# cocowy1/Cost-Volume-Aggregation-in-Stereo-Matching-Revisited

Hardware: AMD Instinct MI355X
Metric: cost-volumes/sec (fwd+bwd) at 544x960 D=192 (higher is better)
Workload: dtype f32

## Files before the change

### cost-volume-aggregation-in-stereo-matching-revisited_amd/csrc/conv3d_c1.hip

```cpp
#include "dca_common.h"
#include "../../include/dca_hip.h"

namespace {
constexpr int TD = 4, TH = 8, TW = 32, CK = 4;
constexpr int ID = TD + 2, IH = TH + 2, IWP = 40;

struct C1Args {
  const float* x;
  const float* w;
  const float* dy;
  float* out;
  int N, C, D, H, W;
  int nTD, nTH, nTW, ntiles;
  int vec;
};

__device__ __forceinline__ void stage_tile(const float* __restrict__ src, float* lds, int n, int C, int c0, int nch,
                                           int D, int H, int W, int d0, int h0, int w0, int vec, int tid) {
  const int rows = nch * ID * IH;
  if (vec) {
    for (int it = tid; it < rows * 8; it += 256) {
      const int row = it >> 3, q = it & 7;
      const int c = row / (ID * IH), rem = row % (ID * IH), id = rem / IH, ih = rem % IH;
      const int ci = c0 + c, d = d0 - 1 + id, h = h0 - 1 + ih, wq = w0 + 4 * q;
// ... 20 lines not shown
      if (ci < C && (unsigned)d < (unsigned)D && (unsigned)h < (unsigned)H && (unsigned)wi < (unsigned)W)
        v = src[((((long)n * C + ci) * D + d) * H + h) * W + wi];
      lds[row * IWP + 3 + j] = v;
    }
  }
}

__device__ __forceinline__ void tile_coords(const C1Args& a, int tile, int& n, int& d0, int& h0, int& w0) {
  const int tw = tile % a.nTW; tile /= a.nTW;
  const int th = tile % a.nTH; tile /= a.nTH;
  const int td = tile % a.nTD;
  n = tile / a.nTD;
  d0 = td * TD; h0 = th * TH; w0 = tw * TW;
}

__global__ __launch_bounds__(256) void c1_bwd_data_kernel(C1Args a) {
  __shared__ __attribute__((aligned(16))) float dy_lds[ID * IH * IWP];
  extern __shared__ __attribute__((aligned(16))) float w_lds[];
  const int tid = threadIdx.x, wq = tid & 7, row = tid >> 3, dl = row >> 3, hl = row & 7;
  int n, d0, h0, w0;
  tile_coords(a, xcd_remap(blockIdx.x, gridDim.x), n, d0, h0, w0);
  stage_tile(a.dy, dy_lds, n, 1, 0, 1, a.D, a.H, a.W, d0, h0, w0, a.vec, tid);
  for (int i = tid; i < a.C * 27; i += 256) {
    const int c = i / 27, t = i % 27;
    w_lds[(c * 9 + t / 3) * 4 + t % 3] = a.w[c * 27 + 26 - t];
  }
  __syncthreads();
  float g[9][6];
#pragma unroll
  for (int r9 = 0; r9 < 9; ++r9) {
    const float* p = dy_lds + ((dl + r9 / 3) * IH + hl + r9 % 3) * IWP + 4 * wq;
    const float4 v = *(const float4*)(p + 4);
    g[r9][0] = p[3]; g[r9][1] = v.x; g[r9][2] = v.y; g[r9][3] = v.z; g[r9][4] = v.w; g[r9][5] = p[8];
  }
  const int d = d0 + dl, h = h0 + hl, w = w0 + 4 * wq;
  const bool ok = d < a.D && h < a.H && w < a.W;
  for (int c = 0; c < a.C; ++c) {
    float acc[4] = {0.f, 0.f, 0.f, 0.f};
#pragma unroll
    for (int r9 = 0; r9 < 9; ++r9) {
      const float4 wv = *(const float4*)(w_lds + (c * 9 + r9) * 4);
#pragma unroll
      for (int j = 0; j < 4; ++j)
        acc[j] = fmaf(wv.z, g[r9][j + 2], fmaf(wv.y, g[r9][j + 1], fmaf(wv.x, g[r9][j], acc[j])));
    }
    if (ok) {
      float* o = a.out + ((((long)n * a.C + c) * a.D + d) * a.H + h) * a.W + w;
      if (a.vec) {
        *(float4*)o = make_float4(acc[0], acc[1], acc[2], acc[3]);
      } else {
#pragma unroll
        for (int j = 0; j < 4; ++j)
          if (w + j < a.W) o[j] = acc[j];
      }
    }
  }
}

__global__ __launch_bounds__(256) void c1_gather_kernel(const float* __restrict__ T, float* __restrict__ y, int D, int H,
                                                        int W) {
  const long DHW = (long)D * H * W;
  const long n = blockIdx.y;
  const float* p = T + n * 27 * DHW;
  const long end = min(DHW, ((long)blockIdx.x + 1) * 1024);
  for (long idx = (long)blockIdx.x * 1024 + threadIdx.x; idx < end; idx += 256) {
    const int w = idx % W;
    const int t = (int)(idx / W);
    const int h = t % H, d = t / H;
    float s = 0.f;
#pragma unroll
// ... 53 lines not shown
      for (int j = 0; j < 4; ++j) v[j] = dca_bload1(dr, base + 4 * j, okr & (int)((unsigned)(w0 + j) < (unsigned)W));
    }
    *(float4*)(out + 4 * (long)q) = make_float4(v[0], v[1], v[2], v[3]);
  }
}

int fill_args(C1Args& a, int N, int C, int D, int H, int W, const void* p0, const void* p1, const void* p2) {
  a.N = N; a.C = C; a.D = D; a.H = H; a.W = W;
  a.nTD = cdiv(D, TD); a.nTH = cdiv(H, TH); a.nTW = cdiv(W, TW);
  const long nt = (long)N * a.nTD * a.nTH * a.nTW;
  if (nt >= (1L << 31)) return 1;
  a.ntiles = (int)nt;
  a.vec = (W % 4 == 0) && ((((uintptr_t)p0 | (uintptr_t)p1 | (uintptr_t)p2) & 15) == 0);
  return 0;
}
}

extern "C" int dca_conv3d_c1_bwd_data(const float* dy, const float* w, float* dx, int N, int C, int D, int H, int W,
                                      hipStream_t stream) {
  DCA_REQUIRE(dy && w && dx && N > 0 && C > 0 && C <= 256 && D > 0 && H > 0 && W > 0);
  C1Args a;
  a.x = nullptr; a.w = w; a.dy = dy; a.out = dx;
  DCA_REQUIRE(fill_args(a, N, C, D, H, W, dy, dx, nullptr) == 0);
  hipLaunchKernelGGL(c1_bwd_data_kernel, dim3(a.ntiles), dim3(256), (size_t)C * 36 * 4, stream, a);
  return dca_launch_status();
}

extern "C" int dca_conv3d_c1_gather(const float* T, float* y, int N, int D, int H, int W, hipStream_t stream) {
  DCA_REQUIRE(T && y && N > 0 && D > 0 && H > 0 && W > 0);
  DCA_REQUIRE(9L * D * H * W * 4 < 0x7ffffff0L && N <= 65535);
// ... 15 lines not shown
```

### cost-volume-aggregation-in-stereo-matching-revisited_amd/csrc/dca_common.h

```cpp
#pragma once
#include <hip/hip_runtime.h>
#include <stdint.h>
#include "../../include/dca_hip.h"

typedef float f32x16 __attribute__((ext_vector_type(16)));
typedef float f32x4 __attribute__((ext_vector_type(4)));

#define DCA_WAVE 64

#define DCA_REQUIRE(cond)                      \
  do {                                         \
    if (!(cond)) return (int)hipErrorInvalidValue; \
  } while (0)

static inline int dca_launch_status() { return (int)hipGetLastError(); }

static inline int cdiv(long a, long b) { return (int)((a + b - 1) / b); }

static inline int dca_num_cus() {
  int dev = 0, v = 0;
  if (hipGetDevice(&dev) == hipSuccess && hipDeviceGetAttribute(&v, hipDeviceAttributeMultiprocessorCount, dev) == hipSuccess &&
      v > 0)
    return v;
  return 256;
}
static inline int dca_persistent_grid(long tiles, int share) {
  const int ncu = dca_num_cus(), g = ncu > share ? ncu / share : 1;
  return (int)(tiles < g ? tiles : g);
}
int dca_internal_wgrad_reduce(const float* part, float* dw, int nblk, int nCxT, int nCT, int K, int Cy, int Cx, long s_cy,
                              long s_cx, hipStream_t stream);

__device__ __forceinline__ int xcd_remap(int bid, int nwg) {
  const int q = nwg >> 3, r = nwg & 7, xcd = bid & 7, idx = bid >> 3;
  const int base = (xcd < r) ? xcd * (q + 1) : r * (q + 1) + (xcd - r) * q;
  return base + idx;
}

__device__ __forceinline__ float act_apply(float v, float slope) { return v > 0.f ? v : v * slope; }

__device__ __forceinline__ float wave_sum(float v) {
#pragma unroll
  for (int o = 32; o > 0; o >>= 1) v += __shfl_xor(v, o, 64);
  return v;
}
__device__ __forceinline__ double wave_sum_d(double v) {
#pragma unroll
  for (int o = 32; o > 0; o >>= 1) v += __shfl_xor(v, o, 64);
  return v;
}
__device__ __forceinline__ float wave_max(float v) {
#pragma unroll
  for (int o = 32; o > 0; o >>= 1) v = fmaxf(v, __shfl_xor(v, o, 64));
  return v;
// ... 65 lines not shown
```

### cost-volume-aggregation-in-stereo-matching-revisited_amd/csrc/dca_frag.h

```cpp
#pragma once
#include "dca_common.h"

typedef __bf16 bf16x8 __attribute__((ext_vector_type(8)));
typedef _Float16 f16x8 __attribute__((ext_vector_type(8)));
typedef _Float16 f16x4 __attribute__((ext_vector_type(4)));
typedef short s16x4 __attribute__((__vector_size__(4 * sizeof(short))));
typedef short s16x8 __attribute__((__vector_size__(8 * sizeof(short))));
typedef __attribute__((address_space(3))) s16x4 lds_s16x4;

template <typename MT> struct Lp;
template <> struct Lp<__bf16> {
  typedef bf16x8 vec8;
  static __device__ __forceinline__ f32x16 mfma(vec8 a, vec8 b, f32x16 c) {
    return __builtin_amdgcn_mfma_f32_32x32x16_bf16(a, b, c, 0, 0, 0);
  }
};
template <> struct Lp<_Float16> {
  typedef f16x8 vec8;
  static __device__ __forceinline__ f32x16 mfma(vec8 a, vec8 b, f32x16 c) {
    return __builtin_amdgcn_mfma_f32_32x32x16_f16(a, b, c, 0, 0, 0);
  }
};
template <typename MT> __device__ __forceinline__ unsigned short lp_bits(float v) {
  const MT m = (MT)v;
// ... 8 lines not shown
template <typename MT> __device__ __forceinline__ float lp_hi(unsigned w) {
  return (float)__builtin_bit_cast(MT, (unsigned short)(w >> 16));
}
template <typename MT> __device__ __forceinline__ unsigned lp_pack2(float a, float b) {
  typedef float f32x2 __attribute__((ext_vector_type(2)));
  typedef MT mtx2 __attribute__((ext_vector_type(2)));
  const f32x2 v = {a, b};
  return __builtin_bit_cast(unsigned, __builtin_convertvector(v, mtx2));
}

__device__ __forceinline__ void x2_split(float v, int e, _Float16& h, _Float16& l) {
  const float u = ldexpf(v, e);
  h = (_Float16)u;
  l = (_Float16)(u - (float)h);
}

__device__ __forceinline__ void x2_prep_exps(int* xe, int A, const unsigned* __restrict__ slots, int nslots,
                                             int* __restrict__ xexps, int xexps_given) {
  const int tid = threadIdx.x;
  if (slots && !xexps_given) {
    for (int c0 = 0; c0 < A; c0 += 32) {
      const int c = c0 + (tid >> 4), l = tid & 15;
      unsigned v = 0;
      if (c < A)
        for (int i = l; i < nslots; i += 16) { const unsigned u = slots[(long)c * DCA_AMAX_CSLOTS + i]; v = v > u ? v : u; }
#pragma unroll
      for (int o = 8; o > 0; o >>= 1) { const unsigned u = (unsigned)__shfl_xor((int)v, o, 64); v = v > u ? v : u; }
      if (c < A && l == 0) {
        const int e = x2_scale_exp(v);
        xe[c] = e;
// ... 96 lines not shown
```

### cost-volume-aggregation-in-stereo-matching-revisited_amd/csrc/pointwise.hip

```cpp
#include "dca_frag.h"
#include "../../include/dca_hip.h"

__global__ __launch_bounds__(256) void bn_stats_kernel(const float* __restrict__ x, double* __restrict__ part, int N,
                                                       int C, long S, int nchunk, long chunk_len, int vec) {
  const int c = blockIdx.x, ch = blockIdx.y, tid = threadIdx.x;
  const long s0 = ch * chunk_len, s1 = min(S, s0 + chunk_len);
  const float K = x[(long)c * S];
  if (ch == 0 && tid == 0) part[(long)C * nchunk * 2 + c] = (double)K;
  float s = 0.f, ss = 0.f;
  for (int n = 0; n < N; ++n) {
    const float* p = x + ((long)n * C + c) * S;
    if (vec) {
      for (long i = s0 + 4 * tid; i < s1; i += 1024) {
        float4 v = *(const float4*)(p + i);
        v.x -= K; v.y -= K; v.z -= K; v.w -= K;
        s += (v.x + v.y) + (v.z + v.w);
        ss += (v.x * v.x + v.y * v.y) + (v.z * v.z + v.w * v.w);
      }
    } else {
      for (long i = s0 + tid; i < s1; i += 256) {
        const float v = p[i] - K;
        s += v;
        ss += v * v;
      }
// ... 135 lines not shown
        const float yv = y[base + i];
        ym = fmaxf(ym, fabsf(yv - mean));
        float v = yv * sc + sh;
        if (res_pre) v += res_pre[base + i];
        v = act_apply(v, slope);
        if (res_post) v += res_post[base + i];
        z[base + i] = v;
        am = fmaxf(am, fabsf(v));
      }
    }
  }
  if (zmax) dca_cmax_put(am, zmax + (long)c * DCA_AMAX_CSLOTS + ch);
  if (ymax) dca_cmax_put(ym, ymax + (long)c * DCA_AMAX_CSLOTS + ch);
}

__device__ __forceinline__ void px2_split(float v, int e, unsigned short& h, unsigned short& l) {
  _Float16 hh, ll;
  x2_split(v, e, hh, ll);
  h = __builtin_bit_cast(unsigned short, hh);
  l = __builtin_bit_cast(unsigned short, ll);
}
typedef unsigned short u16x8 __attribute__((ext_vector_type(8)));

__global__ __launch_bounds__(256) void bn_apply_pack_kernel(const float* __restrict__ y, const float* __restrict__ stats,
                                                            const int* __restrict__ zexps, char* __restrict__ zp, int N,
                                                            int C, long S, long chunk_len, float slope,
                                                            unsigned* __restrict__ ymax, const float* __restrict__ res_pre,
                                                            const float* __restrict__ res_post, float* __restrict__ zf,
                                                            unsigned* __restrict__ zmax) {
  const int cg = blockIdx.y, ch = blockIdx.x, tid = threadIdx.x;
  const long s0 = ch * chunk_len, s1 = min(S, s0 + chunk_len);
  float mean[8], sc[8], sh[8], ym[8], zm[8];
  int ex[8];
#pragma unroll
  for (int j = 0; j < 8; ++j) {
    const int c = cg * 8 + j;
    mean[j] = stats ? stats[c] : 0.f;
    sc[j] = stats ? stats[2 * C + c] : 1.f;
// ... 278 lines not shown
    k1[j] = training ? dca_coherent_loadf(dgb + 2 * C + c) : 0.f;
    k2[j] = training ? dca_coherent_loadf(dgb + 3 * C + c) * stats[C + c] : 0.f;
    ex[j] = dca_coherent_loadi(dyexps + c);
  }
  const long tb = px2_term_bytes(C, S);
  for (int n = 0; n < N; ++n) {
    const long base = ((long)n * C + cg * 8) * S;
    char* ob = dyp + (long)n * 2 * tb + (long)cg * S * 16;
    for (long i = s0 + tid; i < s1; i += 256) {
      float yv[8], dv[8];
#pragma unroll
      for (int j = 0; j < 8; ++j) { yv[j] = y[base + j * S + i]; dv[j] = dz[base + j * S + i]; }
      u16x8 hv, lv;
#pragma unroll
      for (int j = 0; j < 8; ++j) {
        const float u = yv[j] * sc[j] + sh[j];
        const float g = dv[j] * (u > 0.f ? 1.f : slope);
        const float o = (g - k1[j] - (yv[j] - mean[j]) * k2[j]) * sc[j];
        unsigned short h, l;
        px2_split(o, ex[j], h, l);
        hv[j] = h; lv[j] = l;
      }
      *(u16x8*)(ob + i * 16) = hv;
      *(u16x8*)(ob + tb + i * 16) = lv;
    }
  }
}

__global__ __launch_bounds__(256) void avgpool3d_fwd_kernel(const float* __restrict__ x, float* __restrict__ y, int Di,
                                                            int Hi, int Wi, int Do, int Ho, int Wo) {
  const long row = blockIdx.x;
  const int od = (int)(row % Do);
  const long nc = row / Do;
// ... 488 lines not shown
}

extern "C" int dca_bn_backward_reduce(const float* dz, const float* y, const float* stats, double* part, float* dgb, int N,
                                      int C, long S, float slope, int training, hipStream_t stream) {
  DCA_REQUIRE(dz && y && stats && part && dgb && N > 0 && C > 0 && S > 0 && C <= 65535);
  int nchunk; long len;
  chunking(S, C, &nchunk, &len);
  const int vec = (S % 4 == 0) && ((((uintptr_t)dz | (uintptr_t)y) & 15) == 0);
  hipLaunchKernelGGL(bn_bwd_reduce_kernel, dim3(C, nchunk), dim3(256), 0, stream, dz, y, (const float*)nullptr, stats, part,
                     N, C, S, nchunk, len, slope, vec, (unsigned*)nullptr);
  hipLaunchKernelGGL(bn_bwd_finalize_kernel, dim3(C), dim3(64), 0, stream, part, nchunk, (double)N * (double)S, dgb, C,
                     stats, training, (const unsigned*)nullptr, (const unsigned*)nullptr, 0, (int*)nullptr);
  return dca_launch_status();
}

extern "C" int dca_bn_backward_pack(const float* dz, const float* y, const float* stats, double* part, float* dgb, void* dyp,
                                    int* dyexps, unsigned* gmax, const unsigned* ymax, int ymax_slots, int N, int C, long S,
                                    float slope, int training, hipStream_t stream) {
  DCA_REQUIRE(dz && y && stats && part && dgb && dyp && dyexps && gmax && N > 0 && C > 0 && C % 8 == 0 && S > 0 && C <= 65535);
  DCA_REQUIRE((ymax == nullptr || (ymax_slots > 0 && ymax_slots <= DCA_AMAX_CSLOTS)) && ((((uintptr_t)dyp) & 15) == 0));
  int nchunk; long len;
  chunking(S, C, &nchunk, &len);
  const uintptr_t al = (uintptr_t)dz | (uintptr_t)y;
  const int vec = (S % 4 == 0) && ((al & 15) == 0);
  hipLaunchKernelGGL(bn_bwd_reduce_kernel, dim3(C, nchunk), dim3(256), 0, stream, dz, y, (const float*)nullptr, stats, part,
                     N, C, S, nchunk, len, slope, vec, gmax);
  hipLaunchKernelGGL(bn_bwd_finalize_kernel, dim3(C), dim3(64), 0, stream, part, nchunk, (double)N * (double)S, dgb, C,
                     stats, training, (const unsigned*)gmax, ymax, ymax_slots, dyexps);
  int pchunk; long plen;
  chunking(S, C / 8, &pchunk, &plen);
// ... 66 lines not shown
```

### cost-volume-aggregation-in-stereo-matching-revisited_amd/models/augment/cva.py

```python
import torch
import torch.nn as nn

from .._bootstrap import ensure as _ensure
from ..submodule import ConvBn3d, ConvBnReLU3d, conv3d_plain, convbn_3d
from .semantic_level import SemanticLevelContext

ops = _ensure().ops


class _DeconvBn3d(nn.Sequential):

    def __init__(self, cin, cout):
        super().__init__(nn.ConvTranspose3d(cin, cout, 3, padding=1, output_padding=1, stride=2, bias=False),
                         nn.BatchNorm3d(cout))

    def forward(self, x, slope=1.0, res_pre=None, res_post=None, pack_out=False):
        return ops.convbn3d(x, self[0], self[1], slope, res_pre, res_post, pack_out=pack_out)


class Multi_Aggregation(nn.Module):

    def __init__(self, in_channels):
        super().__init__()
        self.conv1 = ConvBnReLU3d(in_channels, in_channels * 2, 3, 2, 1)
# ... 14 lines not shown
        super().__init__(nn.AvgPool3d((3, 3, 3), stride=2, padding=1), ConvBn3d(32, 32, 3, 1, 1),
                         nn.ReLU(inplace=True))

    def forward(self, x):
        return self[1](ops.avg_pool3d_k3s2p1(x), slope=0.0)


class _Classify(nn.Sequential):

    def __init__(self, c):
        super().__init__(ConvBn3d(c, c, 3, 1, 1), nn.ReLU(inplace=True),
                         nn.Conv3d(c, 1, kernel_size=3, padding=1, stride=1, bias=False))

    def forward(self, x, alias=False):
        if alias:
            h, xa = self[0](x, slope=0.0, alias=True)
            return conv3d_plain(h, self[2]), xa
        h = self[0](x, slope=0.0)
        if h.dtype != torch.float32:
            return ops.conv3d_c1_lp(h, self[2].weight)
        return conv3d_plain(h, self[2])


class cva(nn.Module):

    def __init__(self, max_disp, in_channel, downsample=True):
        super().__init__()
        self.max_disp = max_disp
        self.channel = in_channel
        if downsample:
            self.downsample = _Downsample()
        self.slc_net = SemanticLevelContext(feats_channels=self.channel, transform_channels=self.channel,
# ... 44 lines not shown
```

### cost-volume-aggregation-in-stereo-matching-revisited_amd/ops.py

```python
from __future__ import annotations

import ctypes
import math
import os
import threading
from typing import Optional

import torch

from . import _lib

_C = _lib.CONSTANTS
_vp = ctypes.c_void_p


def _L():
    return _lib.load()


def _ptr(t: Optional[torch.Tensor]):
    return _vp(t.data_ptr()) if t is not None else None


_raw_stream = getattr(torch._C, "_cuda_getCurrentRawStream", None)
# ... 256 lines not shown


def _round_up(a, m):
    return (a + m - 1) // m * m


_CONV_MODE = os.environ.get("DCA_CONV", "x2")
CONV_X3 = _CONV_MODE != "fp32"
CONV_X2 = _CONV_MODE == "x2"
WGRAD_S2_X2 = os.environ.get("DCA_WGRAD_S2", "x2") != "fp32"
DECONV_X3 = os.environ.get("DCA_DECONV", "x3") != "fp32"
C1_WGRAD_FUSED = os.environ.get("DCA_C1_WGRAD", "fused") != "expand"
CONV_S2_X2 = os.environ.get("DCA_CONV_S2", "x2") != "fp32"
BN_FUSE = os.environ.get("DCA_BN_FUSE", "1") != "0"
C1_BWD_FUSE = os.environ.get("DCA_C1_BWD", "fused") != "split"
_X3_MIN_WORKGROUPS = 1


AMAX_STATS = {"tagged": 0, "computed": 0, "packed": 0}
CSLOTS = _C["DCA_AMAX_CSLOTS"]
AMAX_EMIT = os.environ.get("DCA_AMAX_EMIT", "1") != "0"
PACK = os.environ.get("DCA_PACK", "1") != "0"


def _cslots(C, device):
    if not AMAX_EMIT:
        return None
    return torch.empty((C * CSLOTS,), device=device, dtype=torch.int32)


# ... 141 lines not shown


def _c1_bwd_route(x, x2, weight, res_pre=None):
    if not C1_BWD_FUSE or res_pre is not None or weight.dim() != 5 or weight.shape[2] != 1 or not torch.is_grad_enabled():
        return "split"
    C1, C2 = x.shape[1], (0 if x2 is None else x2.shape[1])
    if weight.shape[0] != 32 or (C1, C2) not in ((32, 0), (32, 32)) or weight.shape[1] != C1 + C2:
        return "split"
    tensors = (x, weight) if x2 is None else (x, x2, weight)
    if not all(t.is_cuda and t.dtype == torch.float32 and t.requires_grad for t in tensors):
        return "split"
    if x2 is not None and x2.shape != x.shape:
        return "split"
    S = x[0, 0].numel()
    return "fused" if (S % 4 == 0 and x.shape[0] * 32 * S * 4 < 0x7ffff000) else "split"


def _c1_bwd_fused(dz, x, x2, weight):
    tag = getattr(dz, "_dca_lazy", None)
    if tag is None:
        raise RuntimeError("conv3d.backward: expected the gradient the BatchNorm behind this 1x1x1 convolution hands on "
                           "(the tag was lost on the way through autograd)")
    y, stats, dgb, slope, training = tag
    if y.shape != dz.shape or y.shape[0] != x.shape[0] or y.shape[2:] != x.shape[2:]:
        raise RuntimeError("conv3d.backward: the BatchNorm's gradient does not belong to this convolution")
    N, C1 = x.shape[0], x.shape[1]
    C2 = 0 if x2 is None else x2.shape[1]
    S = x[0, 0].numel()
    lib = _L()
    part = torch.empty((lib.dca_conv1_bwd_fused_workspace(N, S, int(x2 is not None)),), device=x.device, dtype=torch.float32)
# ... 556 lines not shown
                dy = torch.empty_like(y)
                want_g = has_pre and slope != 1.0 and ctx.needs_input_grad[9]
                g_out = torch.empty_like(y) if want_g else None
                dm = _cslots(C, y.device) if CONV_X2 else None
                _chk(lib.dca_bn_backward(_ptr(dz), _ptr(y), _ptr(res_pre), _ptr(stats), _ptr(part), _ptr(dgb), _ptr(dy),
                                         _ptr(g_out), N, C, S, float(slope), int(training), _ptr(dm), _stream()),
                     "dca_bn_backward")
                _tag_cmax(dy, dm, nchunk)
        g_pre = None
        if has_pre and ctx.needs_input_grad[9]:
            g_pre = g_out if g_out is not None else dz
        g_post = dz if (has_post and ctx.needs_input_grad[10]) else None
        return dy, dgb[:C], dgb[C:2 * C], None, None, None, None, None, None, g_pre, g_post, None, None, None, None, None


_tls = threading.local()


class frozen_weights:

    def __enter__(self):
        self.prev = getattr(_tls, "frozen", None)
        _tls.frozen = {}
        return self

    def __exit__(self, *exc):
        _tls.frozen = self.prev
        return False


# ... 81 lines not shown

class batched_bn_counters:

    def __enter__(self):
        self.prev = getattr(_tls, "pending", None)
        _tls.pending = []
        return self

    def __exit__(self, *exc):
        pending, _tls.pending = _tls.pending, self.prev
        if pending:
            torch._foreach_add_(pending, 1)
        return False


def bn_act(y, bn, slope=1.0, res_pre=None, res_post=None, stats_part=None, pack_out=False, pack_dy=False, lazy_dy=False):
    momentum = 0.1 if bn.momentum is None else bn.momentum
    training = bn.training or bn.running_mean is None
    if _lp_dtype() is not None:
        raise RuntimeError("ops.reduced_precision is inference only: call the model in eval mode under torch.no_grad()")
    C = y.shape[1]
    pack_z = 0
    if pack_out and PACK and CONV_X2 and training and C % 8 == 0 and torch.is_grad_enabled():
        pack_z = 2 if pack_out == "both" else 1
    pack_dy = bool(pack_dy and PACK and CONV_X2 and res_pre is None and C % 8 == 0)
    zm = _cslots(C, y.device) if (CONV_X2 and pack_z != 1) else None
    z = _BnAct.apply(y, bn.weight, bn.bias, bn.running_mean, bn.running_var, training, momentum, bn.eps, float(slope),
                     res_pre, res_post, stats_part if training else None, zm, pack_z, pack_dy,
                     bool(lazy_dy and res_pre is None))
    if bn.training and bn.num_batches_tracked is not None:
        pending = getattr(_tls, "pending", None)
        if pending is not None:
            pending.append(bn.num_batches_tracked)
        else:
            bn.num_batches_tracked.add_(1)
    return z


class reduced_precision:

    def __init__(self, dtype):
        if dtype not in LP_DTYPES:
            raise ValueError("reduced_precision: torch.bfloat16 or torch.float16")
        self.dtype = dtype

    def __enter__(self):
        self.prev = getattr(_tls, "lp", None)
        _tls.lp = self.dtype
        return self

# ... 46 lines not shown
                                      res_pre, res_post, x2)
    if BN_FUSE and bn.training and conv.weight.shape[0 if not transposed else 1] > 1 and _lp_dtype() is None:
        pdy = _pack_dy_ok(x, x2, conv, transposed, stride, res_pre)
        lazy = not transposed and _c1_bwd_route(x, x2, conv.weight, res_pre) == "fused"
        y, part = _Conv3d.apply(x, x2, conv.weight, int(stride), bool(transposed), True, False, pdy, lazy)
        return bn_act(y, bn, slope, res_pre, res_post, part if part.numel() else None, pack_out=pack_out, pack_dy=pdy,
                      lazy_dy=lazy)
    if not transposed and _lp_dtype() is None and _c1_bwd_route(x, x2, conv.weight, res_pre) == "fused":
        y = _Conv3d.apply(x, x2, conv.weight, int(stride), False, False, False, False, True)
        return bn_act(y, bn, slope, res_pre, res_post, lazy_dy=True)
    if _is_packed(x) and _pack_dy_ok(x, x2, conv, transposed, stride, res_pre):
        y = _Conv3d.apply(x, x2, conv.weight, int(stride), bool(transposed), False, False, True)
        return bn_act(y, bn, slope, res_pre, res_post, pack_dy=True)
    y = conv3d(x, conv.weight, stride, transposed, x2)
    return bn_act(y, bn, slope, res_pre, res_post)


class _AvgPool3d(torch.autograd.Function):
    @staticmethod
    def forward(ctx, x):
        x = _req(x, "avg_pool3d")
        N, C, D, H, W = x.shape
        y = torch.empty((N, C, (D + 1) // 2, (H + 1) // 2, (W + 1) // 2), device=x.device, dtype=torch.float32)
        with torch.cuda.device_of(x):
            _chk(_L().dca_avgpool3d_fwd(_ptr(x), _ptr(y), N * C, D, H, W, _stream()), "dca_avgpool3d_fwd")
        ctx.shape = tuple(x.shape)
        return y

    @staticmethod
    def backward(ctx, gy):
# ... 1008 lines not shown
```

### include/dca_hip.h

```cpp
#ifndef DCA_HIP_H
#define DCA_HIP_H

#include <hip/hip_runtime_api.h>

#ifdef __cplusplus
extern "C" {
#endif

#define DCA_ABI_VERSION 20
int dca_abi_version(void);

#define DCA_BF16 1
#define DCA_FP16 2

int dca_gwc_volume_fwd(const float* ref, const float* tgt, float* vol, int B, int C, int H, int W, int maxdisp,
                       int num_groups, hipStream_t stream);
int dca_gwc_volume_bwd(const float* gvol, const float* ref, const float* tgt, float* gref, float* gtgt, int B, int C,
                       int H, int W, int maxdisp, int num_groups, hipStream_t stream);
int dca_concat_volume_fwd(const float* ref, const float* tgt, float* vol, int B, int C, int H, int W, int maxdisp,
                          hipStream_t stream);
int dca_concat_volume_bwd(const float* gvol, float* gref, float* gtgt, int B, int C, int H, int W, int maxdisp,
                          hipStream_t stream);

int dca_cost_volume_fwd(const float* const* refs, const float* const* tgts, const int* seg_channels, int nseg,
// ... 102 lines not shown
                    int* zexps, const unsigned* rpre_slots, int rpre_n, const unsigned* rpost_slots, int rpost_n, int C,
                    hipStream_t stream);
int dca_bn_apply(const float* y, const float* stats, const float* res_pre, const float* res_post, float* z, int N,
                 int C, long S, float slope, unsigned* zmax, unsigned* ymax, hipStream_t stream);
int dca_bn_apply_pack(const float* y, const float* stats, const int* zexps, void* zp, int N, int C, long S, float slope,
                      unsigned* ymax, const float* res_pre, const float* res_post, float* zf, unsigned* zmax,
                      hipStream_t stream);
int dca_bn_backward(const float* dz, const float* y, const float* res_pre, const float* stats, double* part,
                    float* dgb, float* dy, float* g_out, int N, int C, long S, float slope, int training,
                    unsigned* dmax, hipStream_t stream);
int dca_bn_backward_reduce(const float* dz, const float* y, const float* stats, double* part, float* dgb, int N, int C,
                           long S, float slope, int training, hipStream_t stream);
int dca_bn_backward_pack(const float* dz, const float* y, const float* stats, double* part, float* dgb, void* dyp,
                         int* dyexps, unsigned* gmax, const unsigned* ymax, int ymax_slots, int N, int C, long S,
                         float slope, int training, hipStream_t stream);

int dca_avgpool3d_fwd(const float* x, float* y, long NC, int Di, int Hi, int Wi, hipStream_t stream);
int dca_avgpool3d_bwd(const float* gy, float* gx, const float* res, const float* res2, long NC, int Di, int Hi, int Wi,
                     hipStream_t stream);

int dca_trilinear_fwd(const float* x, float* y, long NC, int Di, int Hi, int Wi, int scale, hipStream_t stream);
int dca_trilinear_bwd(const float* gy, float* gx, long NC, int Di, int Hi, int Wi, int scale, hipStream_t stream);

int dca_context_inject_fwd(const float* x, const float* preds, float* key, int* kstar, float* e, float* pm,
                           float* denom, float* part, int B, int C, int n, long HW, hipStream_t stream);
int dca_context_inject_bwd(const float* dkey, const float* x, const float* preds, const int* kstar, const float* e,
                           const float* pm, const float* denom, float* dx, float* dpreds, float* dw, float* T,
                           float* part, int B, int C, int n, long HW, hipStream_t stream);

int dca_disp_attention_fwd(const float* q, const float* k, const float* v, float* out, int B, int C, int n, long HW,
// ... 139 lines not shown
```

Measured before the change: 43.58.

## Fuse head conv data-grad into BN backward reduce and pack kernels

Adds a fused path for the 32-channel conv+BN+ReLU head followed by the 1-channel 3x3x3 head conv. In backward, the head conv's data gradient is recomputed on the fly from dlogits inside both the BN-backward reduction kernel and the apply/pack kernel, so the full 32-channel dh tensor is never written to or read from memory. The cost is recomputing the 27-tap stencil twice per element and using a fixed-size persistent reduction grid. The path is enabled by default for float32 training.

```diff
diff --git a/cost-volume-aggregation-in-stereo-matching-revisited_amd/csrc/conv3d_c1.hip b/cost-volume-aggregation-in-stereo-matching-revisited_amd/csrc/conv3d_c1.hip
--- a/cost-volume-aggregation-in-stereo-matching-revisited_amd/csrc/conv3d_c1.hip
+++ b/cost-volume-aggregation-in-stereo-matching-revisited_amd/csrc/conv3d_c1.hip
@@ -1,4 +1,4 @@
-#include "dca_common.h"
+#include "dca_frag.h"
 #include "../../include/dca_hip.h"
 
 namespace {
@@ -58,6 +58,31 @@
   d0 = td * TD; h0 = th * TH; w0 = tw * TW;
 }
 
+__device__ __forceinline__ void c1_stage_w(const float* __restrict__ w, float* w_lds, int c0, int nch, int tid) {
+  for (int i = tid; i < nch * 27; i += 256) {
+    const int c = i / 27, t = i % 27;
+    w_lds[(c * 9 + t / 3) * 4 + t % 3] = w[(c0 + c) * 27 + 26 - t];
+  }
+}
+__device__ __forceinline__ void c1_load_row(const float* dy_lds, int dl, int hl, int wq, int r9, float (&g)[6]) {
+  const float* p = dy_lds + ((dl + r9 / 3) * IH + hl + r9 % 3) * IWP + 4 * wq;
+  const float4 v = *(const float4*)(p + 4);
+  g[0] = p[3]; g[1] = v.x; g[2] = v.y; g[3] = v.z; g[4] = v.w; g[5] = p[8];
+}
+__device__ __forceinline__ void c1_load_nbhd(const float* dy_lds, int dl, int hl, int wq, float (&g)[9][6]) {
+#pragma unroll
+  for (int r9 = 0; r9 < 9; ++r9) c1_load_row(dy_lds, dl, hl, wq, r9, g[r9]);
+}
+__device__ __forceinline__ void c1_dx_row(const float4 wv, const float (&g)[6], float (&acc)[4]) {
+#pragma unroll
+  for (int j = 0; j < 4; ++j)
+    acc[j] = fmaf(wv.z, g[j + 2], fmaf(wv.y, g[j + 1], fmaf(wv.x, g[j], acc[j])));
+}
+__device__ __forceinline__ void c1_dx_quad(const float* w_lds, int c, const float (&g)[9][6], float (&acc)[4]) {
+  acc[0] = acc[1] = acc[2] = acc[3] = 0.f;
+#pragma unroll
+  for (int r9 = 0; r9 < 9; ++r9) c1_dx_row(*(const float4*)(w_lds + (c * 9 + r9) * 4), g[r9], acc);
+}
 __global__ __launch_bounds__(256) void c1_bwd_data_kernel(C1Args a) {
   __shared__ __attribute__((aligned(16))) float dy_lds[ID * IH * IWP];
   extern __shared__ __attribute__((aligned(16))) float w_lds[];
@@ -65,29 +90,15 @@
   int n, d0, h0, w0;
   tile_coords(a, xcd_remap(blockIdx.x, gridDim.x), n, d0, h0, w0);
   stage_tile(a.dy, dy_lds, n, 1, 0, 1, a.D, a.H, a.W, d0, h0, w0, a.vec, tid);
-  for (int i = tid; i < a.C * 27; i += 256) {
-    const int c = i / 27, t = i % 27;
-    w_lds[(c * 9 + t / 3) * 4 + t % 3] = a.w[c * 27 + 26 - t];
-  }
+  c1_stage_w(a.w, w_lds, 0, a.C, tid);
   __syncthreads();
   float g[9][6];
-#pragma unroll
-  for (int r9 = 0; r9 < 9; ++r9) {
-    const float* p = dy_lds + ((dl + r9 / 3) * IH + hl + r9 % 3) * IWP + 4 * wq;
-    const float4 v = *(const float4*)(p + 4);
-    g[r9][0] = p[3]; g[r9][1] = v.x; g[r9][2] = v.y; g[r9][3] = v.z; g[r9][4] = v.w; g[r9][5] = p[8];
-  }
+  c1_load_nbhd(dy_lds, dl, hl, wq, g);
   const int d = d0 + dl, h = h0 + hl, w = w0 + 4 * wq;
   const bool ok = d < a.D && h < a.H && w < a.W;
   for (int c = 0; c < a.C; ++c) {
-    float acc[4] = {0.f, 0.f, 0.f, 0.f};
-#pragma unroll
-    for (int r9 = 0; r9 < 9; ++r9) {
-      const float4 wv = *(const float4*)(w_lds + (c * 9 + r9) * 4);
-#pragma unroll
-      for (int j = 0; j < 4; ++j)
-        acc[j] = fmaf(wv.z, g[r9][j + 2], fmaf(wv.y, g[r9][j + 1], fmaf(wv.x, g[r9][j], acc[j])));
-    }
+    float acc[4];
+    c1_dx_quad(w_lds, c, g, acc);
     if (ok) {
       float* o = a.out + ((((long)n * a.C + c) * a.D + d) * a.H + h) * a.W + w;
       if (a.vec) {
@@ -98,6 +109,129 @@
           if (w + j < a.W) o[j] = acc[j];
       }
     }
+  }
+}
+
+struct HeadBwdArgs {
+  C1Args a;
+  const float* stats;
+  float slope;
+  double* part;
+  unsigned* gmax;
+  const float* dgb;
+  const int* dyexps;
+  char* dyp;
+  int training;
+};
+
+__global__ __launch_bounds__(256) void head_bn_reduce_kernel(HeadBwdArgs p) {
+  __shared__ __attribute__((aligned(16))) float dy_lds[ID * IH * IWP];
+  __shared__ __attribute__((aligned(16))) float w_lds[8 * 36];
+  __shared__ double red[4][16];
+  const C1Args& a = p.a;
+  const int tid = threadIdx.x, wq = tid & 7, row = tid >> 3, dl = row >> 3, hl = row & 7, c0 = blockIdx.y * 8;
+  const long DHW = (long)a.D * a.H * a.W;
+  float mean[8], invstd[8], sc[8], sh[8], a0[8], a1[8], gm[8];
+#pragma unroll
+  for (int j = 0; j < 8; ++j) {
+    mean[j] = p.stats[c0 + j]; invstd[j] = p.stats[a.C + c0 + j];
+    sc[j] = p.stats[2 * a.C + c0 + j]; sh[j] = p.stats[3 * a.C + c0 + j];
+    a0[j] = a1[j] = gm[j] = 0.f;
+  }
+  c1_stage_w(a.w, w_lds, c0, 8, tid);
+  const int t0 = (int)((long)blockIdx.x * a.ntiles / gridDim.x), t1 = (int)(((long)blockIdx.x + 1) * a.ntiles / gridDim.x);
+  for (int tile = t0; tile < t1; ++tile) {
+    int n, d0, h0, w0;
+    tile_coords(a, tile, n, d0, h0, w0);
+    __syncthreads();
+    stage_tile(a.dy, dy_lds, n, 1, 0, 1, a.D, a.H, a.W, d0, h0, w0, 1, tid);
+    __syncthreads();
+    const int d = d0 + dl, h = h0 + hl, w = w0 + 4 * wq;
+    if (d < a.D && h < a.H && w < a.W) {
+      float g[9][6];
+      c1_load_nbhd(dy_lds, dl, hl, wq, g);
+      const float* yp = a.x + ((long)n * a.C + c0) * DHW + ((long)d * a.H + h) * a.W + w;
+      float4 yv[8];
+#pragma unroll
+      for (int j = 0; j < 8; ++j) yv[j] = *(const float4*)(yp + j * DHW);
+#pragma unroll
+      for (int j = 0; j < 8; ++j) {
+        float dh[4];
+        c1_dx_quad(w_lds, j, g, dh);
+        const float ys[4] = {yv[j].x, yv[j].y, yv[j].z, yv[j].w};
+#pragma unroll
+        for (int q = 0; q < 4; ++q) {
+          const float gg = bn_bwd_g(dh[q], ys[q], sc[j], sh[j], p.slope);
+          a0[j] += gg;
+          a1[j] += gg * (ys[q] - mean[j]) * invstd[j];
+          gm[j] = fmaxf(gm[j], fabsf(gg));
+        }
+      }
+    }
+  }
+#pragma unroll
+  for (int j = 0; j < 8; ++j) {
+    const double s0 = wave_sum_d((double)a0[j]), s1 = wave_sum_d((double)a1[j]);
+    if ((tid & 63) == 0) { red[tid >> 6][2 * j] = s0; red[tid >> 6][2 * j + 1] = s1; }
+  }
+  __syncthreads();
+  if (tid < 16)
+    p.part[((long)(c0 + (tid >> 1)) * gridDim.x + blockIdx.x) * 2 + (tid & 1)] = red[0][tid] + red[1][tid] + red[2][tid] + red[3][tid];
+#pragma unroll
+  for (int j = 0; j < 8; ++j) dca_cmax_put(gm[j], p.gmax + (long)(c0 + j) * DCA_AMAX_CSLOTS + blockIdx.x);
+}
+
+__global__ __launch_bounds__(256) void head_bn_apply_pack_kernel(HeadBwdArgs p) {
+  __shared__ __attribute__((aligned(16))) float dy_lds[ID * IH * IWP];
+  __shared__ __attribute__((aligned(16))) float w_lds[8 * 36];
+  const C1Args& a = p.a;
+  const int tid = threadIdx.x, wq = tid & 7, row = tid >> 3, dl = row >> 3, hl = row & 7, cg = blockIdx.y, c0 = cg * 8;
+  const long DHW = (long)a.D * a.H * a.W;
+  int n, d0, h0, w0;
+  tile_coords(a, xcd_remap(blockIdx.x, gridDim.x), n, d0, h0, w0);
+  stage_tile(a.dy, dy_lds, n, 1, 0, 1, a.D, a.H, a.W, d0, h0, w0, 1, tid);
+  c1_stage_w(a.w, w_lds, c0, 8, tid);
+  float mean[8], sc[8], sh[8], k1[8], k2[8];
+  int ex[8];
+#pragma unroll
+  for (int j = 0; j < 8; ++j) {
+    const int c = c0 + j;
+    mean[j] = p.stats[c]; sc[j] = p.stats[2 * a.C + c]; sh[j] = p.stats[3 * a.C + c];
+    k1[j] = p.training ? dca_coherent_loadf(p.dgb + 2 * a.C + c) : 0.f;
+    k2[j] = p.training ? dca_coherent_loadf(p.dgb + 3 * a.C + c) * p.stats[a.C + c] : 0.f;
+    ex[j] = dca_coherent_loadi(p.dyexps + c);
+  }
+  __syncthreads();
+  const int d = d0 + dl, h = h0 + hl, w = w0 + 4 * wq;
+  if (!(d < a.D && h < a.H && w < a.W)) return;
+  float g[9][6];
+  c1_load_nbhd(dy_lds, dl, hl, wq, g);
+  const long i = ((long)d * a.H + h) * a.W + w;
+  const float* yp = a.x + ((long)n * a.C + c0) * DHW + i;
+  float4 yv[8];
+#pragma unroll
+  for (int j = 0; j < 8; ++j) yv[j] = *(const float4*)(yp + j * DHW);
+  u16x8 hv[4], lv[4];
+#pragma unroll
+  for (int j = 0; j < 8; ++j) {
+    float dh[4];
+    c1_dx_quad(w_lds, j, g, dh);
+    const float ys[4] = {yv[j].x, yv[j].y, yv[j].z, yv[j].w};
+#pragma unroll
+    for (int q = 0; q < 4; ++q) {
+      const float gg = bn_bwd_g(dh[q], ys[q], sc[j], sh[j], p.slope);
+      const float o = bn_bwd_dy(gg, ys[q], mean[j], k1[j], k2[j], sc[j]);
+      unsigned short hb, lb;
+      px2_split(o, ex[j], hb, lb);
+      hv[q][j] = hb; lv[q][j] = lb;
+    }
+  }
+  const long tb = px2_term_bytes(a.C, DHW);
+  char* ob = p.dyp + (long)n * 2 * tb + (long)cg * DHW * 16 + i * 16;
+#pragma unroll
+  for (int q = 0; q < 4; ++q) {
+    *(u16x8*)(ob + q * 16) = hv[q];
+    *(u16x8*)(ob + tb + q * 16) = lv[q];
   }
 }
 
@@ -181,6 +315,40 @@
   a.vec = (W % 4 == 0) && ((((uintptr_t)p0 | (uintptr_t)p1 | (uintptr_t)p2) & 15) == 0);
   return 0;
 }
+
+int head_reduce_grid(int ntiles) {
+  int g = 2 * dca_num_cus();
+  if (g > DCA_AMAX_CSLOTS) g = DCA_AMAX_CSLOTS;
+  return ntiles < g ? ntiles : g;
+}
+}
+
+extern "C" int dca_bn_backward_pack_head_chunks(int N, int D, int H, int W) {
+  C1Args a;
+  if (N <= 0 || D <= 0 || H <= 0 || W <= 0 || fill_args(a, N, 8, D, H, W, nullptr, nullptr, nullptr)) return 0;
+  return head_reduce_grid(a.ntiles);
+}
+
+extern "C" int dca_bn_backward_pack_head(const float* dlogits, const float* w, const float* y, const float* stats, double* part,
+                                         float* dgb, void* dyp, int* dyexps, unsigned* gmax, const unsigned* ymax,
+                                         int ymax_slots, int N, int C, int D, int H, int W, float slope, int training,
+                                         hipStream_t stream) {
+  DCA_REQUIRE(dlogits && w && y && stats && part && dgb && dyp && dyexps && gmax && N > 0 && C > 0 && C % 8 == 0 && C <= 256 &&
+              D > 0 && H > 0 && W > 0 && W % 4 == 0);
+  DCA_REQUIRE(ymax == nullptr || (ymax_slots > 0 && ymax_slots <= DCA_AMAX_CSLOTS));
+  DCA_REQUIRE(((((uintptr_t)dlogits) | ((uintptr_t)y) | ((uintptr_t)dyp)) & 15) == 0);
+  HeadBwdArgs p;
+  p.a.x = y; p.a.w = w; p.a.dy = dlogits; p.a.out = nullptr;
+  DCA_REQUIRE(fill_args(p.a, N, C, D, H, W, dlogits, y, dyp) == 0 && p.a.vec);
+  p.stats = stats; p.slope = slope; p.part = part; p.gmax = gmax; p.dgb = dgb; p.dyexps = dyexps; p.dyp = (char*)dyp;
+  p.training = training;
+  const int nwg = head_reduce_grid(p.a.ntiles);
+  hipLaunchKernelGGL(head_bn_reduce_kernel, dim3(nwg, C / 8), dim3(256), 0, stream, p);
+  const int rc = dca_internal_bn_bwd_finalize(part, nwg, (double)N * D * H * W, dgb, C, stats, training, gmax, ymax, ymax_slots,
+                                              dyexps, stream);
+  if (rc) return rc;
+  hipLaunchKernelGGL(head_bn_apply_pack_kernel, dim3(p.a.ntiles, C / 8), dim3(256), 0, stream, p);
+  return dca_launch_status();
 }
 
 extern "C" int dca_conv3d_c1_bwd_data(const float* dy, const float* w, float* dx, int N, int C, int D, int H, int W,
diff --git a/cost-volume-aggregation-in-stereo-matching-revisited_amd/csrc/dca_common.h b/cost-volume-aggregation-in-stereo-matching-revisited_amd/csrc/dca_common.h
--- a/cost-volume-aggregation-in-stereo-matching-revisited_amd/csrc/dca_common.h
+++ b/cost-volume-aggregation-in-stereo-matching-revisited_amd/csrc/dca_common.h
@@ -31,6 +31,10 @@
 int dca_internal_wgrad_reduce(const float* part, float* dw, int nblk, int nCxT, int nCT, int K, int Cy, int Cx, long s_cy,
                               long s_cx, hipStream_t stream);
 
+int dca_internal_bn_bwd_finalize(const double* part, int nchunk, double count, float* dgb, int C, const float* stats,
+                                 int training, const unsigned* gmax, const unsigned* ymax, int ymax_slots, int* dyexps,
+                                 hipStream_t stream);
+
 __device__ __forceinline__ int xcd_remap(int bid, int nwg) {
   const int q = nwg >> 3, r = nwg & 7, xcd = bid & 7, idx = bid >> 3;
   const int base = (xcd < r) ? xcd * (q + 1) : r * (q + 1) + (xcd - r) * q;
@@ -38,6 +42,14 @@
 }
 
 __device__ __forceinline__ float act_apply(float v, float slope) { return v > 0.f ? v : v * slope; }
+
+__device__ __forceinline__ float bn_bwd_g(float dz, float y, float sc, float sh, float slope) {
+  const float u = y * sc + sh;
+  return dz * (u > 0.f ? 1.f : slope);
+}
+__device__ __forceinline__ float bn_bwd_dy(float g, float y, float mean, float k1, float k2, float sc) {
+  return (g - k1 - (y - mean) * k2) * sc;
+}
 
 __device__ __forceinline__ float wave_sum(float v) {
 #pragma unroll
diff --git a/cost-volume-aggregation-in-stereo-matching-revisited_amd/csrc/dca_frag.h b/cost-volume-aggregation-in-stereo-matching-revisited_amd/csrc/dca_frag.h
--- a/cost-volume-aggregation-in-stereo-matching-revisited_amd/csrc/dca_frag.h
+++ b/cost-volume-aggregation-in-stereo-matching-revisited_amd/csrc/dca_frag.h
@@ -46,6 +46,13 @@
   h = (_Float16)u;
   l = (_Float16)(u - (float)h);
 }
+__device__ __forceinline__ void px2_split(float v, int e, unsigned short& h, unsigned short& l) {
+  _Float16 hh, ll;
+  x2_split(v, e, hh, ll);
+  h = __builtin_bit_cast(unsigned short, hh);
+  l = __builtin_bit_cast(unsigned short, ll);
+}
+typedef unsigned short u16x8 __attribute__((ext_vector_type(8)));
 
 __device__ __forceinline__ void x2_prep_exps(int* xe, int A, const unsigned* __restrict__ slots, int nslots,
                                              int* __restrict__ xexps, int xexps_given) {
diff --git a/cost-volume-aggregation-in-stereo-matching-revisited_amd/csrc/pointwise.hip b/cost-volume-aggregation-in-stereo-matching-revisited_amd/csrc/pointwise.hip
--- a/cost-volume-aggregation-in-stereo-matching-revisited_amd/csrc/pointwise.hip
+++ b/cost-volume-aggregation-in-stereo-matching-revisited_amd/csrc/pointwise.hip
@@ -173,14 +173,6 @@
   if (ymax) dca_cmax_put(ym, ymax + (long)c * DCA_AMAX_CSLOTS + ch);
 }
 
-__device__ __forceinline__ void px2_split(float v, int e, unsigned short& h, unsigned short& l) {
-  _Float16 hh, ll;
-  x2_split(v, e, hh, ll);
-  h = __builtin_bit_cast(unsigned short, hh);
-  l = __builtin_bit_cast(unsigned short, ll);
-}
-typedef unsigned short u16x8 __attribute__((ext_vector_type(8)));
-
 __global__ __launch_bounds__(256) void bn_apply_pack_kernel(const float* __restrict__ y, const float* __restrict__ stats,
                                                             const int* __restrict__ zexps, char* __restrict__ zp, int N,
                                                             int C, long S, long chunk_len, float slope,
@@ -489,9 +481,8 @@
       u16x8 hv, lv;
 #pragma unroll
       for (int j = 0; j < 8; ++j) {
-        const float u = yv[j] * sc[j] + sh[j];
-        const float g = dv[j] * (u > 0.f ? 1.f : slope);
-        const float o = (g - k1[j] - (yv[j] - mean[j]) * k2[j]) * sc[j];
+        const float g = bn_bwd_g(dv[j], yv[j], sc[j], sh[j], slope);
+        const float o = bn_bwd_dy(g, yv[j], mean[j], k1[j], k2[j], sc[j]);
         unsigned short h, l;
         px2_split(o, ex[j], h, l);
         hv[j] = h; lv[j] = l;
@@ -1010,6 +1001,14 @@
   return dca_launch_status();
 }
 
+int dca_internal_bn_bwd_finalize(const double* part, int nchunk, double count, float* dgb, int C, const float* stats,
+                                 int training, const unsigned* gmax, const unsigned* ymax, int ymax_slots, int* dyexps,
+                                 hipStream_t stream) {
+  hipLaunchKernelGGL(bn_bwd_finalize_kernel, dim3(C), dim3(64), 0, stream, part, nchunk, count, dgb, C, stats, training, gmax,
+                     ymax, ymax_slots, dyexps);
+  return dca_launch_status();
+}
+
 extern "C" int dca_bn_backward_pack(const float* dz, const float* y, const float* stats, double* part, float* dgb, void* dyp,
                                     int* dyexps, unsigned* gmax, const unsigned* ymax, int ymax_slots, int N, int C, long S,
                                     float slope, int training, hipStream_t stream) {
diff --git a/cost-volume-aggregation-in-stereo-matching-revisited_amd/models/augment/cva.py b/cost-volume-aggregation-in-stereo-matching-revisited_amd/models/augment/cva.py
--- a/cost-volume-aggregation-in-stereo-matching-revisited_amd/models/augment/cva.py
+++ b/cost-volume-aggregation-in-stereo-matching-revisited_amd/models/augment/cva.py
@@ -52,8 +52,9 @@
 
     def forward(self, x, alias=False):
         if alias:
-            h, xa = self[0](x, slope=0.0, alias=True)
-            return conv3d_plain(h, self[2]), xa
+            return ops.convbn3d_head(x, self[0][0], self[0][1], self[2], alias=True)
+        if x.dtype == torch.float32 and torch.is_grad_enabled():
+            return ops.convbn3d_head(x, self[0][0], self[0][1], self[2])
         h = self[0](x, slope=0.0)
         if h.dtype != torch.float32:
             return ops.conv3d_c1_lp(h, self[2].weight)
diff --git a/cost-volume-aggregation-in-stereo-matching-revisited_amd/ops.py b/cost-volume-aggregation-in-stereo-matching-revisited_amd/ops.py
--- a/cost-volume-aggregation-in-stereo-matching-revisited_amd/ops.py
+++ b/cost-volume-aggregation-in-stereo-matching-revisited_amd/ops.py
@@ -294,6 +294,7 @@
 CONV_S2_X2 = os.environ.get("DCA_CONV_S2", "x2") != "fp32"
 BN_FUSE = os.environ.get("DCA_BN_FUSE", "1") != "0"
 C1_BWD_FUSE = os.environ.get("DCA_C1_BWD", "fused") != "split"
+HEAD_FUSE = os.environ.get("DCA_HEAD_FUSE", "1") != "0"
 _X3_MIN_WORKGROUPS = 1
 
 
@@ -465,6 +466,26 @@
         return "split"
     S = x[0, 0].numel()
     return "fused" if (S % 4 == 0 and x.shape[0] * 32 * S * 4 < 0x7ffff000) else "split"
+
+
+def _head_route(x, conv, bn, head_conv, alias):
+    if not (HEAD_FUSE and BN_FUSE and torch.is_grad_enabled() and bn.training and _lp_dtype() is None):
+        return "split"
+    if alias and not PAIR_FUSE:
+        return "split"
+    hw = head_conv.weight
+    if bn.weight is None or bn.bias is None or bn.running_mean is None or x.dim() != 5:
+        return "split"
+    if tuple(conv.weight.shape) != (32, 32, 3, 3, 3) or tuple(hw.shape) != (1, 32, 3, 3, 3) or x.shape[1] != 32:
+        return "split"
+    if not all(t.is_cuda and t.dtype == torch.float32 and t.requires_grad for t in (x, conv.weight, bn.weight, bn.bias, hw)):
+        return "split"
+    if not (C1_WGRAD_FUSED and _k3s1(hw, head_conv.stride[0], False, None, head=True)):
+        return "split"
+    N, _, D, H, W = x.shape
+    if W % 4 or N * 32 * D * H * W * 4 >= 0x7ffff000 or not (_is_packed(x) or x.data_ptr() % 16 == 0):
+        return "split"
+    return "fused" if _pack_dy_ok(x, None, conv, False, conv.stride[0], None) else "split"
 
 
 def _c1_bwd_fused(dz, x, x2, weight):
@@ -1051,6 +1072,52 @@
         return dy, dgb[:C], dgb[C:2 * C], None, None, None, None, None, None, g_pre, g_post, None, None, None, None, None
 
 
+class _HeadBnAct(torch.autograd.Function):
+
+    @staticmethod
+    def forward(ctx, y, gamma, beta, running_mean, running_var, momentum, eps, slope, head_w, part):
+        y, head_w = _req(y, "head.batch_norm"), _req(head_w, "head.weight")
+        N, C, D, H, W = y.shape
+        S = D * H * W
+        lib = _L()
+        with torch.cuda.device_of(y):
+            stats = bn_stats_vector(y, gamma, beta, running_mean, running_var, True, momentum, eps, part)
+            ymax = torch.empty((C * CSLOTS,), device=y.device, dtype=torch.int32)
+            h = torch.empty_like(y)
+            _chk(lib.dca_bn_apply(_ptr(y), _ptr(stats), None, None, _ptr(h), N, C, S, float(slope), None, _ptr(ymax), _stream()),
+                 "dca_bn_apply")
+            T = _conv_sliced(h, None, head_w, C, 27, 1, 1, 0, 1, 1, False)
+            logits = torch.empty((N, 1, D, H, W), device=y.device, dtype=torch.float32)
+            _chk(lib.dca_conv3d_c1_gather(_ptr(T), _ptr(logits), N, D, H, W, _stream()), "dca_conv3d_c1_gather")
+        ctx.save_for_backward(y, stats, h, ymax, head_w)
+        ctx.meta = (slope, lib.dca_bn_num_chunks(C, S))
+        return logits
+
+    @staticmethod
+    def backward(ctx, dlogits):
+        y, stats, h, ymax, head_w = ctx.saved_tensors
+        slope, ymax_slots = ctx.meta
+        dlogits = _req(dlogits, "head.backward")
+        N, C, D, H, W = y.shape
+        lib = _L()
+        with torch.cuda.device_of(y):
+            gw = torch.empty_like(head_w)
+            wpart = torch.empty((lib.dca_conv3d_wgrad_workspace(N, C, 27, D, H, W, 1, 1),), device=y.device, dtype=torch.float32)
+            _chk(lib.dca_conv3d_c1_wgrad(_ptr(h), _ptr(dlogits), _ptr(wpart), _ptr(gw), N, C, D, H, W, _stream()),
+                 "dca_conv3d_c1_wgrad")
+            nchunk = lib.dca_bn_backward_pack_head_chunks(N, D, H, W)
+            part = torch.empty((C * nchunk * 2,), device=y.device, dtype=torch.float64)
+            dgb = torch.empty((4 * C,), device=y.device, dtype=torch.float32)
+            dyexps = torch.empty((C,), device=y.device, dtype=torch.int32)
+            gmax = torch.empty((C * CSLOTS,), device=y.device, dtype=torch.int32)
+            dy = torch.empty_like(y)
+            _chk(lib.dca_bn_backward_pack_head(_ptr(dlogits), _ptr(head_w), _ptr(y), _ptr(stats), _ptr(part), _ptr(dgb), _ptr(dy),
+                                               _ptr(dyexps), _ptr(gmax), _ptr(ymax), ymax_slots, N, C, D, H, W, float(slope), 1,
+                                               _stream()), "dca_bn_backward_pack_head")
+            _tag_px2(dy, dyexps)
+        return dy, dgb[:C], dgb[C:2 * C], None, None, None, None, None, gw, None
+
+
 _tls = threading.local()
 
 
@@ -1162,6 +1229,15 @@
         return False
 
 
+def _bn_count(bn):
+    if bn.training and bn.num_batches_tracked is not None:
+        pending = getattr(_tls, "pending", None)
+        if pending is not None:
+            pending.append(bn.num_batches_tracked)
+        else:
+            bn.num_batches_tracked.add_(1)
+
+
 def bn_act(y, bn, slope=1.0, res_pre=None, res_post=None, stats_part=None, pack_out=False, pack_dy=False, lazy_dy=False):
     momentum = 0.1 if bn.momentum is None else bn.momentum
     training = bn.training or bn.running_mean is None
@@ -1176,12 +1252,7 @@
     z = _BnAct.apply(y, bn.weight, bn.bias, bn.running_mean, bn.running_var, training, momentum, bn.eps, float(slope),
                      res_pre, res_post, stats_part if training else None, zm, pack_z, pack_dy,
                      bool(lazy_dy and res_pre is None))
-    if bn.training and bn.num_batches_tracked is not None:
-        pending = getattr(_tls, "pending", None)
-        if pending is not None:
-            pending.append(bn.num_batches_tracked)
-        else:
-            bn.num_batches_tracked.add_(1)
+    _bn_count(bn)
     return z
 
 
@@ -1258,6 +1329,21 @@
         return bn_act(y, bn, slope, res_pre, res_post, pack_dy=True)
     y = conv3d(x, conv.weight, stride, transposed, x2)
     return bn_act(y, bn, slope, res_pre, res_post)
+
+
+def convbn3d_head(x, conv, bn, head_conv, alias=False):
+    if _head_route(x, conv, bn, head_conv, alias) == "split":
+        if alias:
+            h, xa = convbn3d(x, conv, bn, 0.0, alias=True)
+            return conv3d(h, head_conv.weight, head_conv.stride[0], False), xa
+        return conv3d(convbn3d(x, conv, bn, 0.0), head_conv.weight, head_conv.stride[0], False)
+    out = _Conv3d.apply(x, None, conv.weight, 1, False, True, bool(alias), True)
+    y, part = out[0], out[1]
+    momentum = 0.1 if bn.momentum is None else bn.momentum
+    logits = _HeadBnAct.apply(y, bn.weight, bn.bias, bn.running_mean, bn.running_var, momentum, bn.eps, 0.0, head_conv.weight,
+                              part if part.numel() else None)
+    _bn_count(bn)
+    return (logits, out[2]) if alias else logits
 
 
 class _AvgPool3d(torch.autograd.Function):
diff --git a/include/dca_hip.h b/include/dca_hip.h
--- a/include/dca_hip.h
+++ b/include/dca_hip.h
@@ -140,6 +140,10 @@
 int dca_bn_backward_pack(const float* dz, const float* y, const float* stats, double* part, float* dgb, void* dyp,
                          int* dyexps, unsigned* gmax, const unsigned* ymax, int ymax_slots, int N, int C, long S,
                          float slope, int training, hipStream_t stream);
+int dca_bn_backward_pack_head_chunks(int N, int D, int H, int W);
+int dca_bn_backward_pack_head(const float* dlogits, const float* w, const float* y, const float* stats, double* part,
+                              float* dgb, void* dyp, int* dyexps, unsigned* gmax, const unsigned* ymax, int ymax_slots,
+                              int N, int C, int D, int H, int W, float slope, int training, hipStream_t stream);
 
 int dca_avgpool3d_fwd(const float* x, float* y, long NC, int Di, int Hi, int Wi, hipStream_t stream);
 int dca_avgpool3d_bwd(const float* gy, float* gx, const float* res, const float* res2, long NC, int Di, int Hi, int Wi,
```

Measured after the change: 43.77 (median of 6 runs). No clear change (+0.4%).
